# SebastianBitsch/SRGAN-ST

Hardware: AMD Instinct MI355X
Metric: HR images/sec (96px x4, B=16/GPU) G+D+ST-loss step (higher is better)
Workload: dtype f32; 1 GPU; srgan_x4_hr96_b16_G+D+ST-loss step: adv+mse+st, D updated every step (train.py:116-164; BASELINE metric); global_batch=16, hr=96, lr=24, parallelism=dp1, hip_graph=True, d_update_interval=1, d_sr_forward=run: all three discriminator forwards of train.py:136,155,158

## Files before the change

srgan-st_amd/csrc/conv9_c3.hip:

```cpp
#include "conv_common.h"

namespace {

constexpr int TR = 3;
constexpr int TXMAX = 96;
constexpr int MAXU = 9;

struct WgC3Args {
  const float* big;
  const float* small;
  float* slab;
  const float* in_slope;
  float in_slope_const;
  int in_act;
  int kind;
  int B, H, W, C;
  int nrc, nxc;
};

template <int NU>
__global__ __launch_bounds__(CONV_NT, (NU <= 5 ? 2 : 1)) void wgrad_c3_kernel(WgC3Args a) {
  extern __shared__ __attribute__((aligned(16))) float lds[];
  const int tid = threadIdx.x, wave = __builtin_amdgcn_readfirstlane(tid >> 6), lane = tid & 63;
  const int li = lane & 31, lh = lane >> 5;
  const int nfrag = (a.C + 31) >> 5;
  const int CL = nfrag * 32 + 4;
  const int wg = blockIdx.x;
  const int b = wg / (a.nrc * a.nxc), r1 = wg - b * a.nrc * a.nxc;
  const int rc = r1 / a.nxc, xc = r1 - rc * a.nxc;
  const int y0 = rc * TR, x0 = xc * TXMAX;
  const int tw = min(TXMAX, a.W - x0);
  const int RS = (TXMAX + 8) * 3 + 16;
  float* sB = lds;
  float* sS = lds + TXMAX * CL;
  const float slope = a.in_slope ? a.in_slope[0] : a.in_slope_const;
  const int nunits = 9 * nfrag;
  const bool last_ok = wave + 4 * (NU - 1) < nunits;

  for (int i = tid; i < (TR + 8) * RS; i += CONV_NT) {
    const int r = i / RS, o = i - r * RS - 8;
    float v = 0.f;
    const int y = y0 - 4 + r;
    if (o >= 0 && o < (tw + 8) * 3 && (unsigned)y < (unsigned)a.H) {
      const int px = o / 3, ch = o - px * 3, x = x0 - 4 + px;
      if ((unsigned)x < (unsigned)a.W) v = a.small[(((size_t)b * a.H + y) * a.W + x) * 3 + ch];
    }
    sS[i] = v;
  }

  f32x16 acc[NU];
#pragma unroll
  for (int u = 0; u < NU; ++u)
#pragma unroll
    for (int r = 0; r < 16; ++r) acc[u][r] = 0.f;

  int u_fr[NU], u_br[NU];
#pragma unroll
  for (int u = 0; u < NU; ++u) {
    const int unit = wave + 4 * u;
    const int ky = unit / nfrag, fr = unit - ky * nfrag;
    u_fr[u] = fr * 32 + li;
    u_br[u] = (4 + (a.kind ? ky - 4 : 4 - ky)) * RS;
  }
  const int c4n = (nfrag * 32) >> 2;
  const int rows = min(TR, a.H - y0);
  for (int ry = 0; ry < rows; ++ry) {
    const int y = y0 + ry;
    __syncthreads();
    for (int i = tid; i < tw * c4n; i += CONV_NT) {
      const int px = i / c4n, c = (i - px * c4n) * 4;
      f32x4 v = {0.f, 0.f, 0.f, 0.f};
      if (c < a.C) {
        v = *reinterpret_cast<const f32x4*>(a.big + (((size_t)b * a.H + y) * a.W + x0 + px) * a.C + c);
        if (a.in_act == ACT_SLOPE) {
#pragma unroll
          for (int j = 0; j < 4; ++j) v[j] = v[j] > 0.f ? v[j] : v[j] * slope;
        }
      }
      *reinterpret_cast<f32x4*>(&sB[px * CL + c]) = v;
    }
    __syncthreads();
    const int npair = (tw + 1) >> 1;
    if (tw == TXMAX) {
      const float* pa[NU];
      const float* pb[NU];
#pragma unroll
      for (int u = 0; u < NU; ++u) {
        pa[u] = sB + lh * CL + u_fr[u];
        pb[u] = sS + ry * RS + u_br[u] + 8 + 3 * lh + (a.kind ? li : 26 - li);
      }
      float av[NU], bv[NU], an[NU], bn[NU];
#define SST_C3_LOAD(KK, A_, B_)                                                         \
      _Pragma("unroll") for (int u = 0; u < NU; ++u) {                                   \
        if (u < NU - 1 || last_ok) {                                                     \
          A_[u] = pa[u][(KK) * 2 * CL];                                                  \
          B_[u] = pb[u][(KK) * 6];                                                       \
        }                                                                                \
      }
#define SST_C3_MMA(A_, B_)                                                               \
      _Pragma("unroll") for (int u = 0; u < NU; ++u) {                                   \
        if (u < NU - 1 || last_ok) acc[u] = __builtin_amdgcn_mfma_f32_32x32x2f32(A_[u], B_[u], acc[u], 0, 0, 0); \
      }
      constexpr int BLK = 4;
      static_assert((TXMAX / 2) % BLK == 0, "pair blocks");
      SST_C3_LOAD(0, av, bv)
      for (int k0 = 0; k0 < TXMAX / 2; k0 += BLK) {
#pragma unroll
        for (int kk = 0; kk < BLK; kk += 2) {
          SST_C3_LOAD(kk + 1, an, bn)
          SST_C3_MMA(av, bv)
          if (kk + 2 < BLK) { SST_C3_LOAD(kk + 2, av, bv) }
          else if (k0 + BLK < TXMAX / 2) { SST_C3_LOAD(BLK, av, bv) }
          SST_C3_MMA(an, bn)
        }
#pragma unroll
        for (int u = 0; u < NU; ++u) {
          pa[u] += BLK * 2 * CL;
          pb[u] += BLK * 6;
        }
      }
#undef SST_C3_LOAD
#undef SST_C3_MMA
      continue;
    }
    float av[NU], bv[NU];
    auto load_pair = [&](int kk, float (&A)[NU], float (&Bv)[NU]) {
      const int px = 2 * kk + lh;
      const bool pv = px < tw;
      const int so = 8 + 3 * px + (a.kind ? li : 26 - li);
#pragma unroll
      for (int u = 0; u < NU; ++u) {
        if (u < NU - 1 || last_ok) {
          A[u] = pv ? sB[px * CL + u_fr[u]] : 0.f;
          Bv[u] = pv ? sS[ry * RS + u_br[u] + so] : 0.f;
        }
      }
    };
    float an[NU], bn[NU];
    load_pair(0, av, bv);
    for (int kk = 0; kk < npair; kk += 2) {
      load_pair(kk + 1 < npair ? kk + 1 : npair - 1, an, bn);
#pragma unroll
      for (int u = 0; u < NU; ++u) {
        if (u < NU - 1 || last_ok) acc[u] = __builtin_amdgcn_mfma_f32_32x32x2f32(av[u], bv[u], acc[u], 0, 0, 0);
      }
      load_pair(kk + 2 < npair ? kk + 2 : npair - 1, av, bv);
      if (kk + 1 < npair) {
#pragma unroll
        for (int u = 0; u < NU; ++u) {
          if (u < NU - 1 || last_ok) acc[u] = __builtin_amdgcn_mfma_f32_32x32x2f32(an[u], bn[u], acc[u], 0, 0, 0);
        }
      }
    }
  }
  float* out = a.slab + (size_t)wg * 9 * a.C * 32;
#pragma unroll
  for (int u = 0; u < NU; ++u) {
    const int unit = wave + 4 * u;
    if (unit < nunits) {
      const int ky = unit / nfrag, fr = unit - ky * nfrag;
#pragma unroll
      for (int r = 0; r < 16; ++r) {
        const int ch = fr * 32 + (r & 3) + 8 * (r >> 2) + 4 * lh;
        if (ch < a.C) out[((size_t)ky * a.C + ch) * 32 + li] = acc[u][r];
      }
    }
  }
}

__global__ __launch_bounds__(256) void c3_reduce_kernel(const float* __restrict__ slab, float* __restrict__ dw, int nwg, int C,
                                                        int kind, int accumulate) {
  __shared__ f32x4 part[16][16];
  const int item = threadIdx.x & 15, sg = threadIdx.x >> 4;
  const int total4 = 9 * C * 8;
  const int i4 = blockIdx.x * 16 + item;
  f32x4 t = {0.f, 0.f, 0.f, 0.f};
  if (i4 < total4) {
    const f32x4* src = reinterpret_cast<const f32x4*>(slab) + i4;
#pragma unroll 8
    for (int w = sg; w < nwg; w += 16) t += src[(size_t)w * total4];
  }
  part[sg][item] = t;
  __syncthreads();
  if (sg == 0 && i4 < total4) {
#pragma unroll
    for (int g = 1; g < 16; ++g) t += part[g][item];
    const int q0 = (i4 & 7) * 4, ch = (i4 >> 3) % C, ky = (i4 >> 3) / C;
#pragma unroll
    for (int e = 0; e < 4; ++e) {
      const int q = q0 + e;
      if (q >= 27) continue;
      int co, ci;
      const int kx = q / 3;
      if (kind == 0) {
        co = 3 * kx + 2 - q;
        ci = ch;
      } else {
        ci = q - 3 * kx;
        co = ch;
      }
      const int Cin = kind == 0 ? C : 3;
      float* d = dw + (((size_t)co * Cin + ci) * 9 + ky) * 9 + kx;
      *d = accumulate ? *d + t[e] : t[e];
    }
  }
}

}

SST_API int sst_wgrad_c3_supported(int C, int ksize) { return ksize == 9 && C >= 4 && (C & 3) == 0 && C <= 32 * 4 * MAXU / 9; }

SST_API int64_t sst_wgrad_c3_slab_floats(int B, int H, int W, int C) {
  const int nrc = (H + TR - 1) / TR, nxc = (W + TXMAX - 1) / TXMAX;
  return (int64_t)B * nrc * nxc * 9 * C * 32;
}

SST_API int sst_wgrad_c3(const float* big, const float* small, float* slab, float* dw, const float* in_slope,
                         float in_slope_const, int in_act, int kind, int B, int H, int W, int C, int accumulate,
                         void* stream) {
  SST_REQUIRE(big && small && slab && dw && B > 0 && H > 0 && W > 0, "sst_wgrad_c3: bad argument");
  SST_REQUIRE(sst_wgrad_c3_supported(C, 9), "sst_wgrad_c3: C=%d not supported", C);
  SST_REQUIRE(kind == 0 || kind == 1, "sst_wgrad_c3: kind");
  WgC3Args a;
  a.big = big; a.small = small; a.slab = slab; a.in_slope = in_slope; a.in_slope_const = in_slope_const; a.in_act = in_act;
  a.kind = kind; a.B = B; a.H = H; a.W = W; a.C = C;
  a.nrc = (H + TR - 1) / TR;
  a.nxc = (W + TXMAX - 1) / TXMAX;
  const int nfrag = (C + 31) / 32;
  const int nwg = B * a.nrc * a.nxc;
  const size_t smem = ((size_t)TXMAX * (nfrag * 32 + 4) + (size_t)(TR + 8) * ((TXMAX + 8) * 3 + 16)) * sizeof(float);
  const int nu = (9 * nfrag + 3) / 4;
  static bool attr_set = false;
  if (!attr_set) {
    (void)hipFuncSetAttribute(reinterpret_cast<const void*>(wgrad_c3_kernel<3>), hipFuncAttributeMaxDynamicSharedMemorySize, 150 * 1024);
    (void)hipFuncSetAttribute(reinterpret_cast<const void*>(wgrad_c3_kernel<5>), hipFuncAttributeMaxDynamicSharedMemorySize, 150 * 1024);
    (void)hipFuncSetAttribute(reinterpret_cast<const void*>(wgrad_c3_kernel<7>), hipFuncAttributeMaxDynamicSharedMemorySize, 150 * 1024);
    (void)hipFuncSetAttribute(reinterpret_cast<const void*>(wgrad_c3_kernel<9>), hipFuncAttributeMaxDynamicSharedMemorySize, 150 * 1024);
    attr_set = true;
  }
  hipStream_t st = sst_stream(stream);
  if (nu <= 3) wgrad_c3_kernel<3><<<nwg, CONV_NT, smem, st>>>(a);
  else if (nu <= 5) wgrad_c3_kernel<5><<<nwg, CONV_NT, smem, st>>>(a);
  else if (nu <= 7) wgrad_c3_kernel<7><<<nwg, CONV_NT, smem, st>>>(a);
  else wgrad_c3_kernel<9><<<nwg, CONV_NT, smem, st>>>(a);
  SST_LAUNCH_CHECK("wgrad_c3_kernel");
  c3_reduce_kernel<<<(9 * C * 8 + 15) / 16, 256, 0, sst_stream(stream)>>>(slab, dw, nwg, C, kind, accumulate);
  SST_LAUNCH_CHECK("c3_reduce_kernel");
  return SST_OK;
}

namespace {

constexpr int F_TW = 32, F_TH = 4;
constexpr int F_RS = (F_TW + 8) * 3 + 24;

struct C3FwdArgs {
  const float* x;
  const float* wp;
  float* y;
  const float* bias;
  int B, H, W, Cout;
};

__global__ __launch_bounds__(CONV_NT) void conv9_c3_fwd_kernel(C3FwdArgs a) {
  __shared__ float sS[(F_TH + 8) * F_RS];
  const int tid = threadIdx.x, wave = __builtin_amdgcn_readfirstlane(tid >> 6), lane = tid & 63;
  const int li = lane & 31, lh = lane >> 5;
  const int tiles_x = (a.W + F_TW - 1) / F_TW, tiles_y = (a.H + F_TH - 1) / F_TH;
  const int mt = blockIdx.x;
  const int b = mt / (tiles_x * tiles_y), rt = mt - b * tiles_x * tiles_y;
  const int y0 = (rt / tiles_x) * F_TH, x0 = (rt % tiles_x) * F_TW;
  const int nf = blockIdx.y;
  const float* wblk = a.wp + (size_t)nf * 36 * 256 + lane * 4;

  int p_i = 0;
  auto pf_load = [&]() {
    const f32x4 v = *reinterpret_cast<const f32x4*>(wblk + (size_t)(p_i < 36 ? p_i : 35) * 256);
    ++p_i;
    return v;
  };
  f32x4 A0 = pf_load(), A1 = pf_load(), A2 = pf_load(), B0, B1, B2;

  for (int i = tid; i < (F_TH + 8) * F_RS; i += CONV_NT) {
    const int r = i / F_RS, o = i - r * F_RS;
    float v = 0.f;
    const int y = y0 - 4 + r;
    if (o < (F_TW + 8) * 3 && (unsigned)y < (unsigned)a.H) {
      const int px = o / 3, ch = o - px * 3, x = x0 - 4 + px;
      if ((unsigned)x < (unsigned)a.W) v = a.x[(((size_t)b * a.H + y) * a.W + x) * 3 + ch];
    }
    sS[i] = v;
  }
  __syncthreads();

  f32x16 acc;
#pragma unroll
  for (int r = 0; r < 16; ++r) acc[r] = 0.f;
  int a_off = wave * F_RS + 3 * li + 4 * lh, a_c4 = 0;
  auto a_load = [&]() {
    f32x4 v;
#pragma unroll
    for (int j = 0; j < 4; ++j) v[j] = sS[a_off + j];
    const bool wrap = (a_c4 == 3);
    a_off += wrap ? F_RS - 24 : 8;
    a_c4 = wrap ? 0 : a_c4 + 1;
    return v;
  };
#define SST_C3_CHUNK(BUSE, BLOAD)                                                                      \
  {                                                                                                    \
    const f32x4 av = a_load();                                                                         \
    _Pragma("unroll") for (int j = 0; j < 4; ++j)                                                      \
        acc = __builtin_amdgcn_mfma_f32_32x32x2f32(av[j], BUSE[j], acc, 0, 0, 0);                      \
    BLOAD = pf_load();                                                                                 \
  }
  for (int c = 0; c < 36; c += 6) {
    SST_C3_CHUNK(A0, B0)
    SST_C3_CHUNK(A1, B1)
    SST_C3_CHUNK(A2, B2)
    SST_C3_CHUNK(B0, A0)
    SST_C3_CHUNK(B1, A1)
    SST_C3_CHUNK(B2, A2)
  }
#undef SST_C3_CHUNK
  const int oy = y0 + wave, co = nf * 32 + li;
  if (oy < a.H && co < a.Cout) {
    const float bv = a.bias ? a.bias[co] : 0.f;
#pragma unroll
    for (int r = 0; r < 16; ++r) {
      const int ox = x0 + (r & 3) + 8 * (r >> 2) + 4 * lh;
      if (ox < a.W) a.y[(((size_t)b * a.H + oy) * a.W + ox) * a.Cout + co] = acc[r] + bv;
    }
  }
}

__global__ void pack_c3_fwd_kernel(const float* __restrict__ w, float* __restrict__ wp, int Cout, int Cin, int mode) {
  const int total = (int)c3_packed_floats(mode ? Cin : Cout);
  for (int idx = blockIdx.x * blockDim.x + threadIdx.x; idx < total; idx += gridDim.x * blockDim.x)
    wp[idx] = pack_c3_value(w, idx, Cout, Cin, mode);
}

}

SST_API int64_t sst_conv9_c3_packed_floats(int Cout_eff) { return c3_packed_floats(Cout_eff); }

SST_API int sst_conv9_c3_pack(const float* w, float* wp, int Cout, int Cin, int mode, void* stream) {
  SST_REQUIRE(w && wp && Cout > 0 && Cin > 0 && (mode == 0 ? Cin == 3 : Cout == 3), "sst_conv9_c3_pack: the 3-channel side is missing");
  const int O = mode ? Cin : Cout;
  const int total = ((O + 31) / 32) * 36 * 256;
  pack_c3_fwd_kernel<<<(total + 255) / 256, 256, 0, sst_stream(stream)>>>(w, wp, Cout, Cin, mode);
  SST_LAUNCH_CHECK("pack_c3_fwd_kernel");
  return SST_OK;
}

SST_API int sst_conv9_c3_fwd(const float* x, const float* wp, float* y, const float* bias, int B, int H, int W, int Cout,
                             void* stream) {
  SST_REQUIRE(x && wp && y && B > 0 && H > 0 && W > 0 && Cout > 0, "sst_conv9_c3_fwd: bad argument");
  C3FwdArgs a;
  a.x = x; a.wp = wp; a.y = y; a.bias = bias; a.B = B; a.H = H; a.W = W; a.Cout = Cout;
  const int64_t mt = (int64_t)B * ((H + F_TH - 1) / F_TH) * ((W + F_TW - 1) / F_TW);
  SST_REQUIRE(mt < (1ll << 31), "sst_conv9_c3_fwd: too many tiles");
  conv9_c3_fwd_kernel<<<dim3((unsigned)mt, (Cout + 31) / 32), CONV_NT, 0, sst_stream(stream)>>>(a);
  SST_LAUNCH_CHECK("conv9_c3_fwd_kernel");
  return SST_OK;
}

namespace {

constexpr int T3_TH = 8, T3_TW = 24, T3_NT = 512;
constexpr int T3_PW = 32, T3_PH = T3_TH + 8;
constexpr int T3_CB = 32, T3_LDSC = T3_CB + 4;

struct To3Args {
  const float* x;
  const float* wp;
  float* y;
  float* y_pre;
  const float* bias;
  const float* in_slope;
  float in_slope_const;
  int in_act;
  int B, H, W, C;
};

__global__ __launch_bounds__(T3_NT) void conv9_to3_fwd_kernel(To3Args a) {
  extern __shared__ __attribute__((aligned(16))) float lds[];
  const int tid = threadIdx.x, wave = __builtin_amdgcn_readfirstlane(tid >> 6), lane = tid & 63;
  const int li = lane & 31, lh = lane >> 5;
  const int tiles_x = (a.W + T3_TW - 1) / T3_TW, tiles_y = (a.H + T3_TH - 1) / T3_TH;
  const int mt = blockIdx.x;
  const int b = mt / (tiles_x * tiles_y), rt = mt - b * tiles_x * tiles_y;
  const int y0 = (rt / tiles_x) * T3_TH, x0 = (rt % tiles_x) * T3_TW;
  const int ncb = (a.C + CB - 1) / CB;
  const float slope = a.in_slope ? a.in_slope[0] : a.in_slope_const;
  const float* wzero = a.wp + (size_t)ncb * 9 * 8 * 256 + lane * 4;

  f32x16 acc;
#pragma unroll
  for (int r = 0; r < 16; ++r) acc[r] = 0.f;

  for (int pass = 0; pass < 2 * ncb; ++pass) {
    const int cb = pass >> 1, half = pass & 1;
    const int c0 = cb * CB + half * T3_CB;
    if (c0 >= a.C) break;
    const int nks = (min(T3_CB, a.C - c0) + 7) >> 3;
    const int nchunks = 9 * nks;
    const float* wblk = a.wp + (size_t)cb * 9 * 8 * 256 + lane * 4;
    int p_ks = 0, p_off = half * 4 * 256, p_i = 0;
    auto pf_load = [&]() {
      const float* src = p_i < nchunks ? wblk + p_off : wzero;
      const f32x4 v = *reinterpret_cast<const f32x4*>(src);
      const bool wrap = (p_ks + 1 == nks);
      p_ks = wrap ? 0 : p_ks + 1;
      p_off += wrap ? (9 - nks) * 256 : 256;
      ++p_i;
      return v;
    };
    f32x4 A0 = pf_load(), A1 = pf_load(), A2 = pf_load(), B0, B1, B2;
    if (pass) __syncthreads();
    {
      const int c4 = (tid & 7) * 4, c = c0 + c4;
      for (int p = tid >> 3; p < T3_PH * T3_PW; p += T3_NT / 8) {
        const int py = p / T3_PW, px = p - py * T3_PW;
        const int iy = y0 - 4 + py, ix = x0 - 4 + px;
        f32x4 v = {0.f, 0.f, 0.f, 0.f};
        if ((unsigned)iy < (unsigned)a.H && (unsigned)ix < (unsigned)a.W && c < a.C) {
          v = *reinterpret_cast<const f32x4*>(a.x + (((size_t)b * a.H + iy) * a.W + ix) * a.C + c);
          if (a.in_act == ACT_SLOPE) {
#pragma unroll
            for (int j = 0; j < 4; ++j) v[j] = v[j] > 0.f ? v[j] : v[j] * slope;
          }
        }
        *reinterpret_cast<f32x4*>(&lds[p * T3_LDSC + c4]) = v;
      }
    }
    __syncthreads();
    int a_off = (wave * T3_PW + li) * T3_LDSC + 4 * lh, a_ks = 0, a_i = 0;
    auto a_load = [&]() {
      const f32x4 v = *reinterpret_cast<const f32x4*>(&lds[a_off]);
      const bool live = a_i + 1 < nchunks;
      const bool wrap = (a_ks + 1 == nks);
      a_off += live ? (wrap ? T3_PW * T3_LDSC - 8 * (nks - 1) : 8) : 0;
      a_ks = wrap ? 0 : a_ks + 1;
      ++a_i;
      return v;
    };
#define SST_T3_CHUNK(BUSE, BLOAD)                                                                      \
    {                                                                                                  \
      const f32x4 av = a_load();                                                                       \
      _Pragma("unroll") for (int j = 0; j < 4; ++j)                                                    \
          acc = __builtin_amdgcn_mfma_f32_32x32x2f32(av[j], BUSE[j], acc, 0, 0, 0);                    \
      BLOAD = pf_load();                                                                               \
    }
    for (int c = 0; c < nchunks; c += 6) {
      SST_T3_CHUNK(A0, B0)
      SST_T3_CHUNK(A1, B1)
      SST_T3_CHUNK(A2, B2)
      SST_T3_CHUNK(B0, A0)
      SST_T3_CHUNK(B1, A1)
      SST_T3_CHUNK(B2, A2)
    }
#undef SST_T3_CHUNK
  }
  __syncthreads();
  float* sT = lds;
#pragma unroll
  for (int r = 0; r < 16; ++r) sT[(wave * 32 + (r & 3) + 8 * (r >> 2) + 4 * lh) * 33 + li] = acc[r];
  __syncthreads();
  for (int i = tid; i < T3_TH * 3 * T3_TW; i += T3_NT) {
    const int x = i % T3_TW, t = i / T3_TW, co = t % 3, r = t / 3;
    const int oy = y0 + r, ox = x0 + x;
    if (oy < a.H && ox < a.W) {
      float s = a.bias ? a.bias[co] : 0.f;
#pragma unroll
      for (int kx = 0; kx < 9; ++kx) s += sT[(r * 32 + x + kx) * 33 + 3 * kx + co];
      const size_t o = (((size_t)b * 3 + co) * a.H + oy) * a.W + ox;
      if (a.y_pre) a.y_pre[o] = s;
      a.y[o] = fminf(fmaxf(s, 0.f), 1.f);
    }
  }
}

__global__ void pack_to3_kernel(const float* __restrict__ w, float* __restrict__ wp, int C, int64_t total) {
  for (int64_t idx = blockIdx.x * (int64_t)blockDim.x + threadIdx.x; idx < total; idx += (int64_t)gridDim.x * blockDim.x)
    wp[idx] = pack_to3_value(w, idx, C);
}

}

SST_API int64_t sst_conv9_to3_packed_floats(int C) { return to3_packed_floats(C); }

SST_API int sst_conv9_to3_pack(const float* w, float* wp, int C, void* stream) {
  SST_REQUIRE(w && wp && C > 0, "sst_conv9_to3_pack: bad argument");
  const int64_t total = sst_conv9_to3_packed_floats(C);
  pack_to3_kernel<<<(int)((total + 255) / 256), 256, 0, sst_stream(stream)>>>(w, wp, C, total);
  SST_LAUNCH_CHECK("pack_to3_kernel");
  return SST_OK;
}

SST_API int sst_conv9_to3_fwd(const float* x, const float* wp, float* y, float* y_pre, const float* bias, const float* in_slope,
                              float in_slope_const, int in_act, int B, int H, int W, int C, void* stream) {
  SST_REQUIRE(x && wp && y && B > 0 && H > 0 && W > 0 && C > 0 && (C & 3) == 0, "sst_conv9_to3_fwd: bad argument");
  To3Args a;
  a.x = x; a.wp = wp; a.y = y; a.y_pre = y_pre; a.bias = bias; a.in_slope = in_slope; a.in_slope_const = in_slope_const;
  a.in_act = in_act; a.B = B; a.H = H; a.W = W; a.C = C;
  const int64_t mt = (int64_t)B * ((H + T3_TH - 1) / T3_TH) * ((W + T3_TW - 1) / T3_TW);
  SST_REQUIRE(mt < (1ll << 31), "sst_conv9_to3_fwd: too many tiles");
  const size_t smem = (size_t)T3_PH * T3_PW * T3_LDSC * sizeof(float);
  static bool attr_set = false;
  if (!attr_set) {
    (void)hipFuncSetAttribute(reinterpret_cast<const void*>(conv9_to3_fwd_kernel), hipFuncAttributeMaxDynamicSharedMemorySize,
                              (int)smem);
    attr_set = true;
  }
  conv9_to3_fwd_kernel<<<(unsigned)mt, T3_NT, smem, sst_stream(stream)>>>(a);
  SST_LAUNCH_CHECK("conv9_to3_fwd_kernel");
  return SST_OK;
}
```

Baseline: 3257 HR images/s.

## Add multi-row register tiling to 9x9 conv kernels for 3-channel input and output

The 3-channel-input 9x9 forward conv kernel now lets each wave compute several output rows (3 by default when enough workgroups remain). This reuses each loaded weight fragment across more MFMAs and double-buffers the LDS A-operand loads. A new full-row kernel for the 9x9 conv to 3 output channels stages the whole image width per workgroup, prefetches the next channel slice and weights while running MFMAs, and reduces the partial sums over kx in LDS. The cost is more registers, fewer workgroups, and an environment-variable switch that picks between old and new paths.

```diff
diff --git a/srgan-st_amd/csrc/conv9_c3.hip b/srgan-st_amd/csrc/conv9_c3.hip
--- a/srgan-st_amd/csrc/conv9_c3.hip
+++ b/srgan-st_amd/csrc/conv9_c3.hip
@@ -1,4 +1,5 @@
 #include "conv_common.h"
+#include <type_traits>
 
 namespace {
 
@@ -253,6 +254,8 @@
 
 constexpr int F_TW = 32, F_TH = 4;
 constexpr int F_RS = (F_TW + 8) * 3 + 24;
+constexpr int F_ROWS_V2 = 3;
+constexpr int F_V2_MIN_WGS = 512;
 
 struct C3FwdArgs {
   const float* x;
@@ -262,14 +265,16 @@
   int B, H, W, Cout;
 };
 
+template <int ROWS>
 __global__ __launch_bounds__(CONV_NT) void conv9_c3_fwd_kernel(C3FwdArgs a) {
-  __shared__ float sS[(F_TH + 8) * F_RS];
+  constexpr int TH = F_TH * ROWS;
+  __shared__ float sS[(TH + 8) * F_RS];
   const int tid = threadIdx.x, wave = __builtin_amdgcn_readfirstlane(tid >> 6), lane = tid & 63;
   const int li = lane & 31, lh = lane >> 5;
-  const int tiles_x = (a.W + F_TW - 1) / F_TW, tiles_y = (a.H + F_TH - 1) / F_TH;
+  const int tiles_x = (a.W + F_TW - 1) / F_TW, tiles_y = (a.H + TH - 1) / TH;
   const int mt = blockIdx.x;
   const int b = mt / (tiles_x * tiles_y), rt = mt - b * tiles_x * tiles_y;
-  const int y0 = (rt / tiles_x) * F_TH, x0 = (rt % tiles_x) * F_TW;
+  const int y0 = (rt / tiles_x) * TH, x0 = (rt % tiles_x) * F_TW;
   const int nf = blockIdx.y;
   const float* wblk = a.wp + (size_t)nf * 36 * 256 + lane * 4;
 
@@ -281,7 +286,7 @@
   };
   f32x4 A0 = pf_load(), A1 = pf_load(), A2 = pf_load(), B0, B1, B2;
 
-  for (int i = tid; i < (F_TH + 8) * F_RS; i += CONV_NT) {
+  for (int i = tid; i < (TH + 8) * F_RS; i += CONV_NT) {
     const int r = i / F_RS, o = i - r * F_RS;
     float v = 0.f;
     const int y = y0 - 4 + r;
@@ -292,45 +297,71 @@
     sS[i] = v;
   }
   __syncthreads();
-
-  f32x16 acc;
-#pragma unroll
-  for (int r = 0; r < 16; ++r) acc[r] = 0.f;
-  int a_off = wave * F_RS + 3 * li + 4 * lh, a_c4 = 0;
-  auto a_load = [&]() {
-    f32x4 v;
-#pragma unroll
-    for (int j = 0; j < 4; ++j) v[j] = sS[a_off + j];
+  const int oy0 = y0 + wave * ROWS;
+  if (ROWS > 1 && oy0 >= a.H) return;
+
+  f32x16 acc[ROWS];
+#pragma unroll
+  for (int q = 0; q < ROWS; ++q)
+#pragma unroll
+    for (int r = 0; r < 16; ++r) acc[q][r] = 0.f;
+  int a_off = wave * ROWS * F_RS + 3 * li + 4 * lh, a_c4 = 0;
+  auto a_load = [&](f32x4 (&av)[ROWS]) {
+#pragma unroll
+    for (int q = 0; q < ROWS; ++q)
+#pragma unroll
+      for (int j = 0; j < 4; ++j) av[q][j] = sS[a_off + q * F_RS + j];
     const bool wrap = (a_c4 == 3);
     a_off += wrap ? F_RS - 24 : 8;
     a_c4 = wrap ? 0 : a_c4 + 1;
-    return v;
   };
-#define SST_C3_CHUNK(BUSE, BLOAD)                                                                      \
+#define SST_C3_CHUNK(C, AUSE, ALOAD, BUSE, BLOAD)                                                      \
   {                                                                                                    \
-    const f32x4 av = a_load();                                                                         \
+    BLOAD = pf_load();                                                                                 \
+    if ((C) < 35) a_load(ALOAD);                                                                       \
     _Pragma("unroll") for (int j = 0; j < 4; ++j)                                                      \
-        acc = __builtin_amdgcn_mfma_f32_32x32x2f32(av[j], BUSE[j], acc, 0, 0, 0);                      \
-    BLOAD = pf_load();                                                                                 \
-  }
+        _Pragma("unroll") for (int q = 0; q < ROWS; ++q)                                               \
+            acc[q] = __builtin_amdgcn_mfma_f32_32x32x2f32(AUSE[q][j], BUSE[j], acc[q], 0, 0, 0);       \
+    if (ROWS > 1) __builtin_amdgcn_sched_barrier(0);                                                   \
+  }
+  f32x4 av0[ROWS], av1[ROWS];
+  a_load(av0);
+#pragma unroll
   for (int c = 0; c < 36; c += 6) {
-    SST_C3_CHUNK(A0, B0)
-    SST_C3_CHUNK(A1, B1)
-    SST_C3_CHUNK(A2, B2)
-    SST_C3_CHUNK(B0, A0)
-    SST_C3_CHUNK(B1, A1)
-    SST_C3_CHUNK(B2, A2)
+    SST_C3_CHUNK(c, av0, av1, A0, B0)
+    SST_C3_CHUNK(c + 1, av1, av0, A1, B1)
+    SST_C3_CHUNK(c + 2, av0, av1, A2, B2)
+    SST_C3_CHUNK(c + 3, av1, av0, B0, A0)
+    SST_C3_CHUNK(c + 4, av0, av1, B1, A1)
+    SST_C3_CHUNK(c + 5, av1, av0, B2, A2)
   }
 #undef SST_C3_CHUNK
-  const int oy = y0 + wave, co = nf * 32 + li;
-  if (oy < a.H && co < a.Cout) {
+  const int co = nf * 32 + li;
+  if (co < a.Cout) {
     const float bv = a.bias ? a.bias[co] : 0.f;
 #pragma unroll
-    for (int r = 0; r < 16; ++r) {
-      const int ox = x0 + (r & 3) + 8 * (r >> 2) + 4 * lh;
-      if (ox < a.W) a.y[(((size_t)b * a.H + oy) * a.W + ox) * a.Cout + co] = acc[r] + bv;
-    }
-  }
+    for (int q = 0; q < ROWS; ++q) {
+      const int oy = oy0 + q;
+      if (oy >= a.H) break;
+#pragma unroll
+      for (int r = 0; r < 16; ++r) {
+        const int ox = x0 + (r & 3) + 8 * (r >> 2) + 4 * lh;
+        if (ox < a.W) a.y[(((size_t)b * a.H + oy) * a.W + ox) * a.Cout + co] = acc[q][r] + bv;
+      }
+    }
+  }
+}
+
+inline int64_t c3_fwd_wgs(int B, int H, int W, int Cout, int rows) {
+  return (int64_t)B * ((H + F_TH * rows - 1) / (F_TH * rows)) * ((W + F_TW - 1) / F_TW) * ((Cout + 31) / 32);
+}
+
+inline int c3_fwd_rows(int B, int H, int W, int Cout) {
+  if (const char* e = sst_env("SST_C9_V2")) {
+    if (atoi(e) == 0) return 1;
+    if (atoi(e) == 2) return F_ROWS_V2;
+  }
+  return c3_fwd_wgs(B, H, W, Cout, F_ROWS_V2) >= F_V2_MIN_WGS ? F_ROWS_V2 : 1;
 }
 
 __global__ void pack_c3_fwd_kernel(const float* __restrict__ w, float* __restrict__ wp, int Cout, int Cin, int mode) {
@@ -357,9 +388,12 @@
   SST_REQUIRE(x && wp && y && B > 0 && H > 0 && W > 0 && Cout > 0, "sst_conv9_c3_fwd: bad argument");
   C3FwdArgs a;
   a.x = x; a.wp = wp; a.y = y; a.bias = bias; a.B = B; a.H = H; a.W = W; a.Cout = Cout;
-  const int64_t mt = (int64_t)B * ((H + F_TH - 1) / F_TH) * ((W + F_TW - 1) / F_TW);
+  const int rows = c3_fwd_rows(B, H, W, Cout);
+  const int nblk = (Cout + 31) / 32;
+  const int64_t mt = c3_fwd_wgs(B, H, W, Cout, rows) / nblk;
   SST_REQUIRE(mt < (1ll << 31), "sst_conv9_c3_fwd: too many tiles");
-  conv9_c3_fwd_kernel<<<dim3((unsigned)mt, (Cout + 31) / 32), CONV_NT, 0, sst_stream(stream)>>>(a);
+  if (rows == 1) conv9_c3_fwd_kernel<1><<<dim3((unsigned)mt, nblk), CONV_NT, 0, sst_stream(stream)>>>(a);
+  else conv9_c3_fwd_kernel<F_ROWS_V2><<<dim3((unsigned)mt, nblk), CONV_NT, 0, sst_stream(stream)>>>(a);
   SST_LAUNCH_CHECK("conv9_c3_fwd_kernel");
   return SST_OK;
 }
@@ -480,6 +514,166 @@
   }
 }
 
+constexpr int V_R = 6, V_NW = 2 * V_R, V_NT = 64 * V_NW, V_PH = V_R + 8;
+constexpr int V_TS = 27;
+constexpr int V_MAXW = 192;
+constexpr int V_WD = 3;
+
+inline bool to3_rows_applies(int W) { return (W & 31) == 0 && W <= V_MAXW; }
+constexpr size_t to3_rows_smem(int W) {
+  const int nch = W <= 96 ? 2 : 1;
+  const size_t patch = (size_t)V_PH * W * (8 * nch + 4), t = (size_t)nch * V_R * W * V_TS;
+  return (patch > t ? patch : t) * sizeof(float);
+}
+
+template <int NFR>
+__global__ __launch_bounds__(V_NT) void conv9_to3_rows_kernel(To3Args a) {
+  extern __shared__ __attribute__((aligned(16))) float lds[];
+  constexpr int W = 32 * NFR, NCH = NFR <= 3 ? 2 : 1;
+  constexpr int SC = 8 * NCH, ST = SC + 4, C4 = SC / 4;
+  constexpr int PP = 8 / NCH;
+  constexpr int NITEMS = V_PH * W * C4, V_ITEMS = (NITEMS + V_NT - 1) / V_NT;
+  static_assert(V_NT % C4 == 0, "slot per thread");
+  const int tid = threadIdx.x, wave = __builtin_amdgcn_readfirstlane(tid >> 6), lane = tid & 63;
+  const int li = lane & 31, lh = lane >> 5;
+  const int row = wave >> 1, u = wave & 1;
+  const int nrg = (a.H + V_R - 1) / V_R;
+  const int b = blockIdx.x / nrg, y0 = (blockIdx.x - b * nrg) * V_R;
+  const int fb = NCH == 2 ? 0 : 3 * u;
+  const int chs = NCH == 2 ? 8 * u : 0;
+  const int ncb = (a.C + CB - 1) / CB;
+  const float slope = a.in_slope ? a.in_slope[0] : a.in_slope_const;
+  const bool row_ok = y0 + row < a.H;
+
+  const int c_off = (tid % C4) * 4;
+  const int l_off0 = (tid / C4) * ST + c_off;
+  constexpr int L_STEP = (V_NT / C4) * ST;
+  int g_off[V_ITEMS];
+#pragma unroll
+  for (int k = 0; k < V_ITEMS; ++k) {
+    const int i = tid + k * V_NT;
+    const int pp = i / C4;
+    const int py = pp / W, px = pp - py * W;
+    const int iy = y0 - 4 + py;
+    g_off[k] = i < NITEMS && (unsigned)iy < (unsigned)a.H ? ((b * a.H + iy) * W + px) * a.C + c_off : -1;
+  }
+  f32x4 pre[V_ITEMS];
+  auto item_ok = [&](int k, int c0) { return g_off[k] >= 0 && c0 + c_off < a.C; };
+  auto load_pass = [&](int c0) {
+#pragma unroll
+    for (int k = 0; k < V_ITEMS; ++k)
+      pre[k] = *reinterpret_cast<const f32x4*>(a.x + (item_ok(k, c0) ? g_off[k] + c0 : 0));
+  };
+  f32x4 wf[V_WD];
+  auto w_ptr = [&](int ps) {
+    const int cb = ps / PP, p = ps - cb * PP;
+    const int ks = NCH == 2 ? 2 * p + u : p;
+    return a.wp + ((size_t)cb * 9 * 8 + ks) * 256 + lane * 4;
+  };
+
+  f32x16 acc[3];
+#pragma unroll
+  for (int f = 0; f < 3; ++f)
+#pragma unroll
+    for (int r = 0; r < 16; ++r) acc[f][r] = 0.f;
+
+  const int npass = ncb * PP;
+  auto pass_c0 = [&](int ps) { return (ps / PP) * CB + (ps % PP) * SC; };
+  load_pass(0);
+  {
+    const float* src = w_ptr(0);
+#pragma unroll
+    for (int ky = 0; ky < V_WD; ++ky) wf[ky] = *reinterpret_cast<const f32x4*>(src + ky * 8 * 256);
+  }
+  const float* pa = lds + ((size_t)row * W + fb * 32 + li) * ST + chs + 4 * lh;
+  for (int ps = 0; ps < npass; ++ps) {
+    const int c0 = pass_c0(ps);
+    if (c0 >= a.C) break;
+    if (ps) __syncthreads();
+#pragma unroll
+    for (int k = 0; k < V_ITEMS; ++k) {
+      if (tid + k * V_NT < NITEMS) {
+        f32x4 v = pre[k];
+        const bool ok = item_ok(k, c0);
+#pragma unroll
+        for (int j = 0; j < 4; ++j) {
+          v[j] = ok ? v[j] : 0.f;
+          if (a.in_act == ACT_SLOPE) v[j] = v[j] > 0.f ? v[j] : v[j] * slope;
+        }
+        *reinterpret_cast<f32x4*>(&lds[l_off0 + k * L_STEP]) = v;
+      }
+    }
+    __syncthreads();
+    const bool more = ps + 1 < npass && pass_c0(ps + 1) < a.C;
+    const int c0n = more ? pass_c0(ps + 1) : c0;
+    const float* wcur = w_ptr(ps);
+    const float* wnext = w_ptr(more ? ps + 1 : ps);
+    const bool active = row_ok && c0 + chs < a.C;
+    auto run_pass = [&](auto nfc) {
+      constexpr int NF = decltype(nfc)::value;
+#pragma unroll
+      for (int ky = 0; ky < 9; ++ky) {
+        f32x4 av[NF > 0 ? NF : 1];
+#pragma unroll
+        for (int f = 0; f < NF; ++f) av[f] = *reinterpret_cast<const f32x4*>(pa + (ky * W + f * 32) * ST);
+#pragma unroll
+        for (int j = 0; j < 4; ++j)
+#pragma unroll
+          for (int f = 0; f < NF; ++f)
+            acc[f] = __builtin_amdgcn_mfma_f32_32x32x2f32(av[f][j], wf[ky % V_WD][j], acc[f], 0, 0, 0);
+        if (ky == 9 - V_WD) load_pass(c0n);
+        wf[ky % V_WD] = *reinterpret_cast<const f32x4*>(ky + V_WD < 9 ? wcur + (ky + V_WD) * 8 * 256 : wnext + (ky + V_WD - 9) * 8 * 256);
+        __builtin_amdgcn_sched_barrier(0);
+      }
+    };
+    constexpr int NF0 = NCH == 2 ? NFR : 3, NF1 = NCH == 2 ? NFR : NFR - 3;
+    if (!active) run_pass(std::integral_constant<int, 0>{});
+    else if (NF0 == NF1 || u == 0) run_pass(std::integral_constant<int, NF0>{});
+    else run_pass(std::integral_constant<int, NF1>{});
+  }
+  __syncthreads();
+  float* sT = lds;
+  if (li < V_TS) {
+    float* dst = sT + (((NCH == 2 ? u : 0) * V_R + row) * W + fb * 32) * V_TS + li;
+#pragma unroll
+    for (int f = 0; f < 3; ++f)
+      if (fb + f < NFR) {
+#pragma unroll
+        for (int r = 0; r < 16; ++r) dst[(f * 32 + (r & 3) + 8 * (r >> 2) + 4 * lh) * V_TS] = acc[f][r];
+      }
+  }
+  __syncthreads();
+  for (int i = tid; i < V_R * 3 * W; i += V_NT) {
+    const int x = i % W, t = i / W, co = t % 3, r = t / 3;
+    const int oy = y0 + r;
+    if (oy < a.H) {
+      float s = a.bias ? a.bias[co] : 0.f;
+#pragma unroll
+      for (int kx = 0; kx < 9; ++kx) {
+        const int xx = x + kx - 4;
+        if ((unsigned)xx < (unsigned)W) {
+#pragma unroll
+          for (int h = 0; h < NCH; ++h) s += sT[((h * V_R + r) * W + xx) * V_TS + 3 * kx + co];
+        }
+      }
+      const size_t o = (((size_t)b * 3 + co) * a.H + oy) * W + x;
+      if (a.y_pre) a.y_pre[o] = s;
+      a.y[o] = fminf(fmaxf(s, 0.f), 1.f);
+    }
+  }
+}
+
+template <int NFR>
+void to3_rows_launch(const To3Args& a, int64_t nwg, hipStream_t st) {
+  static bool attr_set = false;
+  if (!attr_set) {
+    (void)hipFuncSetAttribute(reinterpret_cast<const void*>(conv9_to3_rows_kernel<NFR>), hipFuncAttributeMaxDynamicSharedMemorySize,
+                              (int)to3_rows_smem(32 * NFR));
+    attr_set = true;
+  }
+  conv9_to3_rows_kernel<NFR><<<(unsigned)nwg, V_NT, to3_rows_smem(32 * NFR), st>>>(a);
+}
+
 __global__ void pack_to3_kernel(const float* __restrict__ w, float* __restrict__ wp, int C, int64_t total) {
   for (int64_t idx = blockIdx.x * (int64_t)blockDim.x + threadIdx.x; idx < total; idx += (int64_t)gridDim.x * blockDim.x)
     wp[idx] = pack_to3_value(w, idx, C);
@@ -503,6 +697,23 @@
   To3Args a;
   a.x = x; a.wp = wp; a.y = y; a.y_pre = y_pre; a.bias = bias; a.in_slope = in_slope; a.in_slope_const = in_slope_const;
   a.in_act = in_act; a.B = B; a.H = H; a.W = W; a.C = C;
+  hipStream_t st = sst_stream(stream);
+  const char* v2 = sst_env("SST_C9_V2");
+  if (to3_rows_applies(W) && !(v2 && atoi(v2) == 0)) {
+    SST_REQUIRE((int64_t)B * H * W * C < (1ll << 31), "sst_conv9_to3_fwd: tensor too large");
+    const int64_t nwg = (int64_t)B * ((H + V_R - 1) / V_R);
+    SST_REQUIRE(nwg < (1ll << 31), "sst_conv9_to3_fwd: too many tiles");
+    switch (W >> 5) {
+      case 1: to3_rows_launch<1>(a, nwg, st); break;
+      case 2: to3_rows_launch<2>(a, nwg, st); break;
+      case 3: to3_rows_launch<3>(a, nwg, st); break;
+      case 4: to3_rows_launch<4>(a, nwg, st); break;
+      case 5: to3_rows_launch<5>(a, nwg, st); break;
+      default: to3_rows_launch<6>(a, nwg, st); break;
+    }
+    SST_LAUNCH_CHECK("conv9_to3_rows_kernel");
+    return SST_OK;
+  }
   const int64_t mt = (int64_t)B * ((H + T3_TH - 1) / T3_TH) * ((W + T3_TW - 1) / T3_TW);
   SST_REQUIRE(mt < (1ll << 31), "sst_conv9_to3_fwd: too many tiles");
   const size_t smem = (size_t)T3_PH * T3_PW * T3_LDSC * sizeof(float);
@@ -512,7 +723,7 @@
                               (int)smem);
     attr_set = true;
   }
-  conv9_to3_fwd_kernel<<<(unsigned)mt, T3_NT, smem, sst_stream(stream)>>>(a);
+  conv9_to3_fwd_kernel<<<(unsigned)mt, T3_NT, smem, st>>>(a);
   SST_LAUNCH_CHECK("conv9_to3_fwd_kernel");
   return SST_OK;
 }
```

Result: no change. 3261 HR images/s, median of 6 (+0.1%).
